# balkce/beamform

Hardware: AMD Instinct MI355X
Metric: stft_frames_per_sec (higher is better)
Workload: dtype f64; 1 GPU; das 8-mic 1024-pt (hop 512), 65536-frame batch per GPU, 1 stream(s), planar input resident in HBM; frames_per_gpu=65536, frames_fed_per_gpu=65536, mics=8, fft=1024, hop=512, streams=1, layout=planar, gather=n/a, parallelism=independent batches x1, input=uniform noise in [-0.5, 0.5), settle_launches_before_warmup=408, forward_transforms_per_frame_pair=6

## Files before the change

beamform_amd/csrc/das_f64_plan.hpp:

```cpp
#pragma once

#include <cstdlib>
#include <cstring>

#if defined(__HIPCC__)
#define BF_PLAN_HD __host__ __device__ inline
#else
#define BF_PLAN_HD inline
#endif

namespace bf {

constexpr int kChunkEnd = 0xFFFFF;
constexpr int kMaxChunkPairs = 1000;
constexpr int kSchedMaxChunks = 16384;

struct DasSchedPlan {
    int n_levels;
    int cnt[8], size[8];
    int n_chunks;
    int grid;
};

BF_PLAN_HD void das_f64_chunk(const DasSchedPlan &p, long n_frames, int n_streams, int k, int *stream, long *t0, long *n) {
    int lvl = 0, kk = k;
    long pair0 = 0;
    while (lvl < p.n_levels - 1 && kk >= p.cnt[lvl] * n_streams) {
        kk -= p.cnt[lvl] * n_streams;
        pair0 += (long)p.cnt[lvl] * p.size[lvl];
        ++lvl;
    }
    const int s = kk / p.cnt[lvl], j = kk - s * p.cnt[lvl];
    *stream = s;
    *t0 = 2 * (pair0 + (long)j * p.size[lvl]);
    long len = 2L * p.size[lvl];
    if (*t0 + len > n_frames) len = n_frames - *t0;
    *n = len;
}

inline DasSchedPlan das_f64_plan(long n_frames, int n_streams, int n_cus, const char *env) {
    DasSchedPlan p{};
    const long pairs = (n_frames + 1) / 2;
    long nb = (long)n_cus / n_streams;
    if (nb < 1) nb = 1;
    int sizes[8], n_sizes = 0;
    const long share = (pairs + nb - 1) / nb;
    if (env && strchr(env, ',')) {
        const char *c = env;
        while (*c && n_sizes < 8) {
            sizes[n_sizes++] = atoi(c);
            c = strchr(c, ',');
            if (!c) break;
            ++c;
        }
    } else if (!(env && atoi(env) == 0) && share >= 48) {
        long front = (share * 13 / 16) & ~7L;
        long rest = share - front;
        while (front > kMaxChunkPairs && n_sizes < 3) {
            sizes[n_sizes++] = kMaxChunkPairs;
            front -= kMaxChunkPairs;
        }
        if (front > kMaxChunkPairs) { rest += front - kMaxChunkPairs; front = kMaxChunkPairs; }
        sizes[n_sizes++] = (int)front;
        while (n_sizes < 6 && rest >= 24) {
            long sz = (rest / 2) & ~7L;
            if (sz > kMaxChunkPairs) sz = kMaxChunkPairs;
            sizes[n_sizes++] = (int)sz;
            rest -= sz;
        }
        if (rest >= 12) { sizes[n_sizes++] = 4; rest -= 4; }
        sizes[n_sizes++] = 2;
// ... 33 lines not shown
```

beamform_amd/csrc/das_f64_w64.hip:

```cpp
#include <hip/hip_runtime.h>

#include <type_traits>

#include "launch_trace.hpp"
#include "pipeline_kernels.hpp"
#include "switches.hpp"
#include "w64_f64_dev.hpp"

namespace bf {

namespace {

constexpr int kBlock = 512;
constexpr int kWaves = kBlock / 64;
constexpr int kHop = 512;
constexpr int kTwD = 2 * (1024 + 4 * kTw2RowW64Rot);
constexpr int oTw = 0;
constexpr int oPlane = kTwD;
constexpr int oGain = oPlane + kWaves * kPlaneD;
constexpr int oCross = oGain + 4 * 2048;
constexpr int oFlag = oCross + 512;
constexpr int kWinRow = 18;
constexpr int oWin = oFlag + 8;
constexpr int kLdsD = oWin + 64 * kWinRow;
// ... 218 lines not shown
                for (int j = 0; j < 8; ++j) atomicAdd(yo + (unsigned)(64 * j + lane), o[j]);
            }
        } else {
            const float *parea = (pw < kWaves - 1) ? reinterpret_cast<const float *>(lds + oPlane + pw * kPlaneD) : s_cross + ((it + 1) & 1) * kHop;
            while (s_ready[pw] < (int)(t - 1)) __builtin_amdgcn_s_sleep(1);
            asm volatile("" ::: "memory");
            float prev[8];
#pragma unroll
            for (int j = 0; j < 8; ++j) prev[j] = parea[64 * j + lane];
            asm volatile("" ::: "memory");
            if (lane == 0) s_cons[pw] = (int)(t - 1);
#pragma unroll
            for (int j = 0; j < 8; ++j) yo[(unsigned)(64 * j + lane)] = prev[j] + o[j];
        }
        if (t == T1 - 1) {
            if (T1 < a.n_frames) {
                float *yn = ys + T1 * kHop;
#pragma unroll
                for (int j = 0; j < 8; ++j) atomicAdd(yn + (unsigned)(64 * j + lane), o[j + 8]);
            } else {
                float *to = a.tail_out + (long)stream * kHop;
#pragma unroll
                for (int j = 0; j < 8; ++j) to[(unsigned)(64 * j + lane)] = o[j + 8];
            }
        }
    }
}


#ifdef BF_PARK_PLAIN
#define BF_PARK_LD(p) (*(const volatile float *)(p))
#else
#define BF_PARK_LD(p) __builtin_nontemporal_load(p)
#endif
constexpr int kGRow = 65;
constexpr int kGMic = 8 * kGRow;
constexpr int kSlots = 64;
constexpr int kTwP = 2 * (960 + 4 * kTw2RowW64Rot);
constexpr int pTw = 0;
constexpr int pPlane = kTwP;
constexpr int pGain = pPlane + kWaves * kPlaneD;
constexpr int pFlag = pGain + 7 * kGMic * 2;
constexpr int kRingR = 32;
constexpr int kRingSlots = kRingR + kWaves;
constexpr int pRing = pFlag + (kSlots + 4) / 2;
constexpr int pWin = pRing + kRingR / 2;
constexpr int kLdsP = pWin + 64 * kWinRow;
static_assert(kLdsP * 8 <= 160 * 1024, "LDS");
static_assert((pGain & 1) == 0 && (pWin & 1) == 0, "16-byte alignment");


typedef volatile __attribute__((address_space(3))) int *lds_int_t;
typedef volatile __attribute__((address_space(3))) unsigned long long *lds_u64_t;
__device__ __forceinline__ int lds_fetch_add(lds_int_t p, int v, int lane) {
    int old = 0;
    if (lane == 0) old = __hip_atomic_fetch_add((__attribute__((address_space(3))) int *)p, v, __ATOMIC_RELAXED, __HIP_MEMORY_SCOPE_WORKGROUP);
    return __builtin_amdgcn_readfirstlane(old);
}
__device__ __forceinline__ unsigned long long lds_fetch_add64(lds_u64_t p, int lane) {
    unsigned long long old = 0;
    if (lane == 0) old = __hip_atomic_fetch_add((__attribute__((address_space(3))) unsigned long long *)p, 1ull, __ATOMIC_RELAXED, __HIP_MEMORY_SCOPE_WORKGROUP);
    const unsigned lo = (unsigned)__builtin_amdgcn_readfirstlane((int)(unsigned)old), hi = (unsigned)__builtin_amdgcn_readfirstlane((int)(unsigned)(old >> 32));
    return ((unsigned long long)hi << 32) | lo;
}
struct DasSched {
    const int4 *chunks;
    unsigned *counter;
    int n_chunks;
};
__device__ __forceinline__ unsigned long long pack_work(unsigned vbase, int chunk, int pairs, int next) {
    return ((unsigned long long)(vbase & 0xFFFFFFu) << 40) | ((unsigned long long)(unsigned)chunk << 20) | ((unsigned long long)(unsigned)pairs << 10) | (unsigned)next;
}
struct PairWork {
    int4 d;
    int pos;
    int len;
    unsigned u;
    bool have;
};
__device__ __forceinline__ int4 load_chunk(const int4 *chunks, int k) {
    const int4 d = chunks[k];
    return int4{__builtin_amdgcn_readfirstlane(d.x), __builtin_amdgcn_readfirstlane(d.y), __builtin_amdgcn_readfirstlane(d.z), k};
}
__device__ __forceinline__ PairWork draw_pair(lds_u64_t work, const DasSched &sc, int lane, const int4 held) {
    PairWork r;
    r.have = false;
    r.d = int4{0, 0, 0, 0};
    r.pos = r.len = 0;
    r.u = 0;
    for (;;) {
        const unsigned long long old = lds_fetch_add64(work, lane);
        const int pos = (int)(old & 1023u), len = (int)((old >> 10) & 1023u), k = (int)((old >> 20) & 0xFFFFFu);
        const unsigned vb = (unsigned)(old >> 40);
        if (k == kChunkEnd) return r;
        if (pos < len) {
            if (k == held.w) r.d = held;
            else r.d = load_chunk(sc.chunks, k);
            r.pos = pos; r.len = len; r.u = vb + (unsigned)pos; r.have = true;
            return r;
        }
        if (pos == len) {
            unsigned k2 = 0;
            if (lane == 0) k2 = __hip_atomic_fetch_add(sc.counter, 1u, __ATOMIC_RELAXED, __HIP_MEMORY_SCOPE_AGENT);
            k2 = (unsigned)__builtin_amdgcn_readfirstlane((int)k2);
            if (k2 >= (unsigned)sc.n_chunks) {
                if (lane == 0) *work = pack_work(vb + (unsigned)len, kChunkEnd, 0, 0);
                return r;
            }
            r.d = load_chunk(sc.chunks, (int)k2);
            r.len = (r.d.z + 1) >> 1;
            r.pos = 0; r.u = vb + (unsigned)len; r.have = true;
            if (lane == 0) *work = pack_work(r.u, (int)k2, r.len, 1);
            return r;
        }
        while ((int)((*work >> 20) & 0xFFFFFu) == k) __builtin_amdgcn_s_sleep(2);
    }
}
__device__ __forceinline__ int claim_boundary(lds_int_t st, unsigned b, int lane) {
    const int base = 4 * (int)(b / kSlots);
    while (st[b & (kSlots - 1)] < base) __builtin_amdgcn_s_sleep(1);
    return lds_fetch_add(st + (b & (kSlots - 1)), 1, lane) - base;
}
__device__ __forceinline__ void publish_boundary(lds_int_t st, unsigned b, int lane) { (void)lds_fetch_add(st + (b & (kSlots - 1)), 2, lane); }
__device__ __forceinline__ void skip_boundary(lds_int_t st, unsigned b, int lane) {
    const int base = 4 * (int)(b / kSlots);
    while (st[b & (kSlots - 1)] < base) __builtin_amdgcn_s_sleep(1);
    (void)lds_fetch_add(st + (b & (kSlots - 1)), 4, lane);
}
__device__ __forceinline__ void await_boundary(lds_int_t st, unsigned b) {
    while (st[b & (kSlots - 1)] - 4 * (int)(b / kSlots) < 3) __builtin_amdgcn_s_sleep(1);
}

#ifdef BF_W64_STATS
__device__ unsigned long long g_stats[256 * 8 * 5];
#define BF_STATS_DECL unsigned long long st_[5] = {0, 0, 0, 0, 0}; const unsigned long long st_t0_ = __builtin_amdgcn_s_memrealtime()
#define BF_STAT(i) (++st_[i])
#define BF_STAT_WAIT_BEGIN const unsigned long long st_w0_ = __builtin_amdgcn_s_memrealtime()
#define BF_STAT_WAIT_END st_[3] += __builtin_amdgcn_s_memrealtime() - st_w0_
#define BF_STATS_FLUSH do { st_[4] = __builtin_amdgcn_s_memrealtime() - st_t0_; if (lane == 0 && blockIdx.x < 256) for (int i_ = 0; i_ < 5; ++i_) g_stats[(blockIdx.x * 8 + w) * 5 + i_] = st_[i_]; } while (0)
#else
#define BF_STATS_DECL
#define BF_STAT(i) ((void)0)
// ... 167 lines not shown
            r.h = ring_slot(jp);
        }
        __builtin_amdgcn_fence(__ATOMIC_ACQUIRE, "workgroup");
        return r;
    };
    auto release_pair = [&](const PairWork &pw, bool has_t) {
        const unsigned u2 = 2u * pw.u;
        (void)lds_fetch_add(s_ring + (u2 & (kRingR - 1)), 2, lane);
        (void)lds_fetch_add(s_ring + ((u2 + 1) & (kRingR - 1)), has_t ? 1 : 2, lane);
        if (pw.pos > 0) (void)lds_fetch_add(s_ring + ((u2 - 1) & (kRingR - 1)), 1, lane);
    };
    auto request_ring_mic = [&](const RingHops &r, int m) { request(r.h + m * kHop, r.a + m * kHop, r.b + m * kHop); };
    auto request_ring_extra = [&](bool on, const RingHops &r) {
        if (!on) {
#pragma unroll
            for (int j = 0; j < 8; ++j) e0[j] = e1[j] = e2[j] = 0.f;
            return;
        }
#pragma unroll
        for (int j = 0; j < 8; ++j) {
            e0[j] = r.h[XM * kHop + (unsigned)(64 * j + lane)];
            e1[j] = r.a[XM * kHop + (unsigned)(64 * j + lane)];
            e2[j] = r.b[XM * kHop + (unsigned)(64 * j + lane)];
        }
    };
    RingHops curR{nullptr, nullptr, nullptr};
    (void)curR;

    BF_STAMP(0);
#ifdef BF_W64_STAMPS
    if (lane == 0 && blockIdx.x < 256) g_stamps[(blockIdx.x * 8 + w) * 64 + 59] = __builtin_amdgcn_s_memtime();
#endif
    PairWork cur;
    cur.d = load_chunk(sc.chunks, (int)blockIdx.x);
    cur.len = (cur.d.z + 1) >> 1;
    const int n_static = cur.len < kWaves ? cur.len : kWaves;
    cur.pos = w;
    cur.u = (unsigned)w;
    cur.have = w < n_static;
    if (LAYOUT == 0 && cur.have) {
        request_pair_mic(cur.d.x, cur.d.y + 2L * w, a.slot_mic[0]);
        request_extra(XM >= 0, cur.d.x, cur.d.y + 2L * w);
    } else {
        request_extra(false, 0, 0);
    }
    {
        const f64x2 *tw2 = a.tw + 64;
        f64x2 *ltw = reinterpret_cast<f64x2 *>(lds + pTw), *lg = reinterpret_cast<f64x2 *>(lds + pGain);
#pragma unroll 4
        for (int i = tid; i < kTwP / 2; i += kBlock) ltw[i] = tw2[i];
        for (int k = 0; k < NT; ++k) {
            const f64x2 *g2 = a.gains_mic + a.slot_mic[k] * kGMic;
#pragma unroll 2
            for (int i = tid; i < kGMic; i += kBlock) lg[k * kGMic + i] = g2[i];
        }
#pragma unroll 2
        for (int i = tid; i < 1024; i += kBlock) lds[pWin + (i & 63) * kWinRow + (i >> 6)] = a.win[i];
        if (tid < kSlots) s_state[tid] = 0;
        if (tid < kRingR) s_ring[tid] = 0;
        if (tid == 0) *s_work = pack_work(0u, (int)blockIdx.x, cur.len, n_static);
    }
    __syncthreads();
    BF_STAMP(1);
    BF_STATS_DECL;
    int it = 0;
    if (!cur.have) {
        cur = draw_pair(s_work, sc, lane, cur.d);
// ... 184 lines not shown
        if (has_t) {
            oT = claim_boundary(s_state, u, lane);
            if (oT == 0) {
#pragma unroll
                for (int j = 0; j < 8; ++j) yn[(unsigned)(64 * j + lane)] = tl[j];
            }
        } else {
            skip_boundary(s_state, u, lane);
        }
#pragma unroll
        for (int j = 0; j < 16; ++j) {
            const float f = (float)Sr[j];
            oA[j] = (float)((double)f * wrow[j]);
        }
        if (pair) {
            float *y1 = ys + (tA + 1) * kHop;
#pragma unroll
            for (int j = 0; j < 8; ++j) {
                const float f0 = (float)Si[j];
                const float b0 = (float)((double)f0 * wrow[j]);
                y1[(unsigned)(64 * j + lane)] = oA[j + 8] + b0;
            }
        }
        if (has_h) {
            oH = claim_boundary(s_state, u - 1, lane);
            if (oH == 0) {
#pragma unroll
                for (int j = 0; j < 8; ++j) yo[(unsigned)(64 * j + lane)] = oA[j];
            }
        } else if (T0 == 0) {
            const float *ti = a.tail_in + (long)stream * kHop;
#pragma unroll
            for (int j = 0; j < 8; ++j) yo[(unsigned)(64 * j + lane)] = ti[(unsigned)(64 * j + lane)] + oA[j];
        } else {
#pragma unroll
            for (int j = 0; j < 8; ++j) atomicAdd(yo + (unsigned)(64 * j + lane), oA[j]);
        }
        if (oT == 0 || oH == 0) {
            __builtin_amdgcn_fence(__ATOMIC_RELEASE, "workgroup");
            if (oT == 0) publish_boundary(s_state, u, lane);
            if (oH == 0) publish_boundary(s_state, u - 1, lane);
        }
        if (oT > 0) {
            BF_STAT(2);
            BF_STAT_WAIT_BEGIN;
            await_boundary(s_state, u);
            BF_STAT_WAIT_END;
            __builtin_amdgcn_fence(__ATOMIC_ACQUIRE, "workgroup");
            float o[8];
#pragma unroll
            for (int j = 0; j < 8; ++j) o[j] = BF_PARK_LD(yn + (unsigned)(64 * j + lane));
#pragma unroll
            for (int j = 0; j < 8; ++j) yn[(unsigned)(64 * j + lane)] = tl[j] + o[j];
        } else {
            BF_STAT(0);
        }
        if (oH > 0) {
            BF_STAT(2);
            BF_STAT_WAIT_BEGIN;
            await_boundary(s_state, u - 1);
            BF_STAT_WAIT_END;
            __builtin_amdgcn_fence(__ATOMIC_ACQUIRE, "workgroup");
            float o[8];
#pragma unroll
            for (int j = 0; j < 8; ++j) o[j] = BF_PARK_LD(yo + (unsigned)(64 * j + lane));
#pragma unroll
            for (int j = 0; j < 8; ++j) yo[(unsigned)(64 * j + lane)] = o[j] + oA[j];
        } else {
            BF_STAT(1);
        }
        if (!has_t) {
            if (T1 < a.n_frames) {
                float *ynx = ys + T1 * kHop;
#pragma unroll
                for (int j = 0; j < 8; ++j) atomicAdd(ynx + (unsigned)(64 * j + lane), tl[j]);
            } else {
                float *to = a.tail_out + (long)stream * kHop;
#pragma unroll
                for (int j = 0; j < 8; ++j) to[(unsigned)(64 * j + lane)] = tl[j];
                if (a.hist_out != nullptr) {
                    float *ho = a.hist_out + (long)stream * M * kHop;
                    const float *xs = a.x + (long)stream * a.stream_stride_x;
                    for (int m = 0; m < M; ++m) {
                        const float *xl = xs + (long)m * a.mic_stride + tL * kHop;
#pragma unroll
                        for (int j = 0; j < 8; ++j) ho[m * kHop + 64 * j + lane] = xl[(unsigned)(64 * j + lane)];
                    }
                }
            }
        }
        if constexpr (LAYOUT == 1) {
            asm volatile("" ::: "memory");
            release_pair(cur, has_t);
        }
        cur = nxt;
        ++it;
    }
    BF_STATS_FLUSH;
#ifdef BF_W64_STAMPS
    if (lane == 0 && blockIdx.x < 256) {
        g_stamps[(blockIdx.x * 8 + w) * 64 + 63] = __builtin_amdgcn_s_memrealtime();
        g_stamps[(blockIdx.x * 8 + w) * 64 + 60] = __builtin_amdgcn_s_memtime();
        g_stamps[(blockIdx.x * 8 + w) * 64 + 62] = (unsigned long long)it;
        g_stamps[(blockIdx.x * 8 + w) * 64 + 61] = (unsigned long long)__builtin_amdgcn_s_getreg(((4 - 1) << 11) | (0 << 6) | 20);
    }
#endif
    (void)it;
}

__global__ __launch_bounds__(kBlock) void das_f64_pair_kernel(DasF64Args a, DasSched sc) { das_f64_pair_body<0>(a, sc); }
__global__ __launch_bounds__(kBlock) void das_f64_ring_kernel(DasF64Args a, DasSched sc) { das_f64_pair_body<1>(a, sc); }

constexpr int kSchedPerBlock = 8;
__global__ __launch_bounds__(32 * kSchedPerBlock) void das_f64_sched_kernel(DasSchedPlan p, int4 *chunks, unsigned *counter, float *y, long n_frames, int n_streams) {
    const int k = blockIdx.x * kSchedPerBlock + (int)(threadIdx.x >> 5), l = (int)(threadIdx.x & 31);
    if (k >= p.n_chunks) return;
    int stream;
    long t0, n;
    das_f64_chunk(p, n_frames, n_streams, k, &stream, &t0, &n);
    if (l == 0) {
        chunks[k] = int4{stream, (int)t0, (int)n, 0};
        if (k == 0) *counter = (unsigned)p.grid;
    }
    if (t0 > 0) {
        float4 *h = reinterpret_cast<float4 *>(y + ((long)stream * n_frames + t0) * kHop);
        for (int i = l; i < kHop / 4; i += 32) h[i] = float4{0.f, 0.f, 0.f, 0.f};
    }
}

__global__ __launch_bounds__(256) void interleaved_to_planar_kernel(const float *x, float *out, long tiles_per_stream, int M, long in_stream_stride,
                                                                    long out_mic_stride, long out_stream_stride) {
    __shared__ float s_t[256 * 9];
    const int tid = threadIdx.x;
    const long s = blockIdx.x / tiles_per_stream, tile = blockIdx.x - s * tiles_per_stream;
    const float4 *src = reinterpret_cast<const float4 *>(x + s * in_stream_stride + tile * 256 * M);
    const int R = M + 1;
    for (int i = tid; i < 64 * M; i += 256) {
        const float4 v = src[i];
        const int e = 4 * i;
        s_t[(e / M) * R + e % M] = v.x;
        s_t[((e + 1) / M) * R + (e + 1) % M] = v.y;
        s_t[((e + 2) / M) * R + (e + 2) % M] = v.z;
        s_t[((e + 3) / M) * R + (e + 3) % M] = v.w;
    }
    __syncthreads();
    float *dst = out + s * out_stream_stride + tile * 256;
    for (int j = tid; j < 64 * M; j += 256) {
        const int m = j >> 6, q = j & 63;
        const float4 v{s_t[(4 * q) * R + m], s_t[(4 * q + 1) * R + m], s_t[(4 * q + 2) * R + m], s_t[(4 * q + 3) * R + m]};
        reinterpret_cast<float4 *>(dst + (long)m * out_mic_stride)[q] = v;
    }
}

}

constexpr size_t kSchedCounterBytes = 256;
size_t das_f64_sched_ws_bytes() { return kSchedCounterBytes + (size_t)kSchedMaxChunks * sizeof(int4); }

DasF64Launch das_f64_decide(int layout, int n_mics, int n_streams, long n_frames, int n_cus, bool mic0_unit, int n_tr, bool tables) {
    DasF64Launch d{};
    if (n_mics > 8) return d;
    const bool ring = switches().das_il_ring != 0 && (n_mics == 2 || n_mics == 4 || n_mics == 8);
    bool frame_pair = tables && mic0_unit && n_mics >= 2 && n_tr >= 1;
    if (layout != BF_PLANAR && !ring && ((n_frames * kHop) & 255) != 0) frame_pair = false;
    if (!frame_pair) {
        if (layout == BF_PLANAR) return d;
        const long runs = n_cus > n_streams ? n_cus / n_streams : 1;
        d.path = DasF64Path::kMicPair;
        d.run_frames = ((n_frames + runs - 1) / runs + kWaves - 1) / kWaves * kWaves;
        d.runs_per_stream = (n_frames + d.run_frames - 1) / d.run_frames;
        return d;
    }
    if ((long)n_streams * ((n_frames + 1) / 2) >= (1L << 31)) return d;
    d.plan = das_f64_plan(n_frames, n_streams, n_cus, switches().das_f64_sched);
    if (d.plan.n_chunks < 1 || d.plan.n_chunks > kSchedMaxChunks) return d;
    d.path = layout == BF_PLANAR ? DasF64Path::kFramePair : ring ? DasF64Path::kRing : DasF64Path::kTranspose;
    d.writes_hist = layout == BF_PLANAR;
    const size_t hop_elems = (size_t)n_mics * kHop;
    d.scratch_bytes = sizeof(float) * (layout == BF_PLANAR ? 0 : ring ? n_cus * kRingSlots * hop_elems : n_streams * hop_elems * (n_frames + 1));
    return d;
}

static hipError_t launch_interleaved_to_planar(const float *x, float *out, long n, int n_mics, int n_streams, hipStream_t s) {
    const long tiles = n / 256;
    BF_LAUNCH(interleaved_to_planar_kernel, dim3((unsigned)(tiles * n_streams)), dim3(256), 0, s, x, out, tiles, n_mics, (long)n_mics * n, n, (long)n_mics * n);
    return hipGetLastError();
}

hipError_t enqueue_das_f64(DasF64Args a, const DasF64Launch &d, float *scratch, hipStream_t s, hipEvent_t kev0, hipEvent_t kev1, bool *kev_recorded) {
    hipError_t e = hipSuccess;
    int4 *const chunks = reinterpret_cast<int4 *>(reinterpret_cast<char *>(a.sched_ws) + kSchedCounterBytes);
    const DasSched sc{chunks, reinterpret_cast<unsigned *>(a.sched_ws), d.plan.n_chunks};
    if (d.path == DasF64Path::kMicPair) {
        for (int st = 0; st < a.n_streams && d.runs_per_stream > 1; ++st) {
            e = hipMemset2DAsync(a.y + ((long)st * a.n_frames + d.run_frames) * kHop, (size_t)d.run_frames * kHop * sizeof(float), 0, kHop * sizeof(float), (size_t)d.runs_per_stream - 1, s);
            if (e != hipSuccess) return e;
        }
    } else {
        if (d.path == DasF64Path::kRing) {
            a.ring = scratch; a.ring_bytes = d.scratch_bytes; a.hist_out = nullptr;
        } else if (d.path == DasF64Path::kTranspose) {
            const long n = a.n_frames * kHop;
            float *const hist = scratch + (size_t)a.n_streams * a.n_mics * n;
            if ((e = launch_interleaved_to_planar(a.x, scratch, n, a.n_mics, a.n_streams, s)) != hipSuccess) return e;
            if ((e = launch_interleaved_to_planar(a.hist, hist, kHop, a.n_mics, a.n_streams, s)) != hipSuccess) return e;
            a.x = scratch; a.hist = hist; a.hist_out = nullptr; a.mic_stride = n; a.layout = BF_PLANAR;
        }
        BF_LAUNCH(das_f64_sched_kernel, dim3((unsigned)((sc.n_chunks + kSchedPerBlock - 1) / kSchedPerBlock)), dim3(32 * kSchedPerBlock), 0, s, d.plan, chunks, sc.counter, a.y, a.n_frames, a.n_streams);
        if ((e = hipGetLastError()) != hipSuccess) return e;
    }
    if (kev0 && (e = hipEventRecord(kev0, s)) != hipSuccess) return e;
    if (d.path == DasF64Path::kMicPair)
        BF_LAUNCH(das_f64_w64_kernel<1>, dim3((unsigned)(d.runs_per_stream * a.n_streams)), dim3(kBlock), 0, s, a, (int)d.run_frames, (int)d.runs_per_stream);
    else if (d.path == DasF64Path::kRing)
        BF_LAUNCH(das_f64_ring_kernel, dim3((unsigned)d.plan.grid), dim3(kBlock), 0, s, a, sc);
    else
        BF_LAUNCH(das_f64_pair_kernel, dim3((unsigned)d.plan.grid), dim3(kBlock), 0, s, a, sc);
    if ((e = hipGetLastError()) != hipSuccess) return e;
    if (kev1 && (e = hipEventRecord(kev1, s)) == hipSuccess) *kev_recorded = true;
    return e;
}

}

#ifdef BF_W64_STATS
extern "C" int bf_dbg_stats(unsigned long long *host) {
    return (int)hipMemcpyFromSymbol(host, HIP_SYMBOL(bf::g_stats), sizeof(unsigned long long) * 256 * 8 * 5);
}
#endif
#ifdef BF_W64_STAMPS
extern "C" int bf_dbg_stamps(unsigned long long *host) {
    return (int)hipMemcpyFromSymbol(host, HIP_SYMBOL(bf::g_stamps), sizeof(unsigned long long) * 256 * 8 * 64);
}
#endif
```

beamform_amd/csrc/pipeline.hip:

```cpp
#include "pipeline.hpp"

#include <hip/hip_runtime.h>

#include <cmath>
#include <vector>

#include "device_mem.hpp"
#include "fft1024.hpp"
#include "pipeline_kernels.hpp"
#include "switches.hpp"

namespace bf {

namespace {

class BinPipelineImpl : public Engine {
    static constexpr int kMaxCols = BF_MAX_INTERF + 1;
   public:
    BinPipelineImpl(const bf_config &c, int n_cus) : cfg_(c), n_cus_(n_cus) {
        M_ = c.n_mics;
        H_ = c.hop;
        N_ = 2 * c.hop;
        NQ_ = problems_per_frame(N_);
        YS_ = yh_stride(N_);
// ... 28 lines not shown
        if (cov_node_ && (Phist_ < 1 || Phist_ > 64)) {
            err_ = "past_windows must be in 1..64";
            return BF_EINVAL;
        }
        if (time_node_ && (M_ > 16 || cfg_.gsc_filter_size < 1 || cfg_.gsc_filter_size > 256)) {
            err_ = "gsc is built for up to 16 microphones and filter_size 1..256";
            return M_ > 16 ? BF_ENOSYS : BF_EINVAL;
        }
        if (cfg_.algo == BF_PHASEMPF && (cfg_.smooth_size < 1 || cfg_.smooth_size > 64)) {
            err_ = "smooth_size must be in 1..64";
            return BF_EINVAL;
        }
        ENGINE_HIP(d_tw_.upload(N_ == 1024 ? twiddle_table_32x32<f64x2>() : stockham_twiddles<f64x2>(N_)));
        ENGINE_HIP(d_tw32_.upload(twiddle_table_32x32<f32x2>()));
        ENGINE_HIP(d_win_.upload(sqrt_hann(N_)));
        freqs_ = frequency_vector(N_, cfg_.sample_rate);
        ENGINE_HIP(d_freq_.upload(freqs_));
        skip_lo_ = N_; band_yh_hi_ = NQ_ - 1;
        if (band_node_) {
            int klo = N_, khi = 0;
            for (int q = 1; q < NQ_; ++q) {
                const double f = std::fabs(freqs_[q]);
                if (f >= cfg_.freq_min && f <= cfg_.freq_max) { if (q < klo) klo = q; khi = q; }
            }
            if (khi < N_ / 2 - 2) { skip_lo_ = khi; skip_hi_ = N_ - khi; }
            if (cov_node_ && khi < N_ / 2 - 1 && klo <= khi) { band_yh_lo_ = klo; band_yh_hi_ = khi; }
            else if (cov_node_ && klo > khi) { band_yh_lo_ = 1; band_yh_hi_ = 0; }
        }
        for (auto &b : d_steer_) ENGINE_HIP(b.alloc(steer_elems()));
        if (das_one_launch_shape()) {
            for (auto &b : d_dasg_w64_) ENGINE_HIP(b.alloc((size_t)4 * 1024));
            for (auto &b : d_dasg_mic_) ENGINE_HIP(b.alloc((size_t)8 * kDasMicGainRows * kDasMicGainRow));
            ENGINE_HIP(d_das_sched_.alloc(das_f64_sched_ws_bytes()));
        }
        if (N_ == 1024) ENGINE_HIP(d_tw_w64_.upload(twiddle_table_w64_rot()));
        for (auto &b : d_hist2_) ENGINE_HIP(b.alloc(hist_elems()));
        for (auto &b : d_tail_) ENGINE_HIP(b.alloc(tail_elems()));
        if (Phist_ > 0) ENGINE_HIP(d_zhist_.alloc(zhist_bytes()));
        if (cfg_.algo == BF_GSS) {
            ENGINE_HIP(d_gssW_.alloc(gss_bytes() / sizeof(f64x2)));
            ENGINE_HIP(hipMemset(d_gssW_.get(), 0, gss_bytes()));
        }
        if (cfg_.algo == BF_PHASEMPF || cfg_.algo == BF_MCRA) ENGINE_HIP(d_mpf_.alloc(mpf_bytes() / sizeof(double)));
        if (cfg_.algo == BF_PHASEMPF) ENGINE_HIP(d_smooth_.alloc(smooth_bytes() / sizeof(double)));
        if (time_node_) ENGINE_HIP(d_nlms_.alloc(nlms_bytes() / sizeof(float)));
        return BF_OK;
    }

    int reset(hipStream_t st) override {
        ENGINE_HIP(hipMemsetAsync(d_hist2_[0].get(), 0, hist_elems() * sizeof(float), st));
        hist_cur_ = 0;
        for (auto &b : d_tail_) ENGINE_HIP(hipMemsetAsync(b.get(), 0, tail_elems() * sizeof(float), st));
        tail_cur_ = 0;
        if (d_zhist_.get()) ENGINE_HIP(hipMemsetAsync(d_zhist_.get(), 0, zhist_bytes(), st));
        if (d_mpf_.get()) ENGINE_HIP(hipMemsetAsync(d_mpf_.get(), 0, mpf_bytes(), st));
        if (d_smooth_.get()) ENGINE_HIP(hipMemsetAsync(d_smooth_.get(), 0, smooth_bytes(), st));
        if (d_nlms_.get()) ENGINE_HIP(hipMemsetAsync(d_nlms_.get(), 0, nlms_bytes(), st));
        gss_reset_mask_ = ~0ull;
        return BF_OK;
    }

    int upload_steering(const std::vector<SteeringSet> &dirs, hipStream_t stream) override {
        const int nc = dirs[0].n_cols, nd = (int)dirs.size();
        if ((size_t)nd * nc * M_ * N_ > steer_elems()) {
            err_ = "steering table larger than the device buffer";
            return BF_EINVAL;
// ... 117 lines not shown
    const bool yraw_target_ = cfg_.algo == BF_PHASEMPF || time_node_;
    int skip_lo_, skip_hi_ = 0;
    int band_yh_lo_ = 0, band_yh_hi_;
    bool z48_ = false;
    size_t zsz_ = sizeof(f64x2);
    int H_ = 512, N_ = 1024, NQ_ = 514, YS_ = 516;
    const KernelSet *ks_ = nullptr;
    long steer_dir_stride_ = 0;
    std::vector<double> freqs_;
    DeviceBuffer<f64x2> d_tw_;
    DeviceBuffer<f32x2> d_tw32_;
    DeviceBuffer<double> d_win_, d_freq_;
    DeviceBuffer<f64x2> d_steer_[2];
    DeviceBuffer<f64x2> d_dasg_w64_[2];
    DeviceBuffer<f64x2> d_tw_w64_;
    DeviceBuffer<char> d_das_sched_;
    DeviceBuffer<f64x2> d_dasg_mic_[2];
    bool das_mic0_unit_[2] = {false, false};
    DasSlots das_slots_[2];
    int steer_cur_ = 0;
    DeviceBuffer<float> d_hist2_[2];
    int hist_cur_ = 0;
    DeviceBuffer<float> d_tail_[2];
    int tail_cur_ = 0;
    DeviceBuffer<char> d_zhist_;
    DeviceBuffer<f64x2> d_gssW_;
    DeviceBuffer<double> d_mpf_;
    DeviceBuffer<double> d_smooth_;
    DeviceBuffer<float> d_nlms_;
    unsigned long long gss_reset_mask_ = ~0ull;
    DeviceBuffer<char> d_Z_;
    DeviceBuffer<char> d_Yh_;
    DeviceBuffer<float> d_yraw_;
    DeviceBuffer<float> d_planar_;
    DeviceBuffer<float> d_frames_;
};

int BinPipelineImpl::run_das_one_launch(const float *x, long F, float *y, hipStream_t stream, int layout, long mic_stride, const RunSnapshot &snap) {
    if (!das_one_launch_shape() || switches().fused_bins != 1 || snap.das_gains_w64 == nullptr) return kDeclined;
    const DasF64Launch d = das_f64_decide(layout, M_, S_, F, n_cus_, snap.das_mic0_unit, snap.das_slots.n_tr,
                                          snap.das_gains_mic != nullptr && d_das_sched_.get() != nullptr);
    if (d.path == DasF64Path::kChain) return kDeclined;
    ENGINE_HIP(d_planar_.reserve((d.scratch_bytes + sizeof(float) - 1) / sizeof(float)));
    float *const hist = d_hist2_[hist_cur_].get();
    DasF64Args da;
    da.x = x; da.hist = hist; da.hist_out = d_hist2_[hist_cur_ ^ 1].get(); da.y = y;
    da.tail_in = d_tail_[tail_cur_].get(); da.tail_out = d_tail_[tail_cur_ ^ 1].get();
    da.win = d_win_.get(); da.n_frames = F; da.mic_stride = mic_stride;
    da.stream_stride_x = (long)M_ * F * H_; da.n_streams = S_; da.n_mics = M_; da.run_len = 1;
    da.layout = layout;
    da.gains = snap.das_gains_w64; da.gains_mic = snap.das_gains_mic; da.tw = d_tw_w64_.get();
    da.mic0_unit = snap.das_mic0_unit ? 1 : 0;
    da.n_tr = snap.das_slots.n_tr; da.extra_mic = snap.das_slots.extra_mic;
    for (int k = 0; k < 8; ++k) da.slot_mic[k] = snap.das_slots.slot_mic[k];
    da.sched_ws = d_das_sched_.get(); da.sched_ws_bytes = d_das_sched_.get() ? das_f64_sched_ws_bytes() : 0;
    ENGINE_HIP(enqueue_das_f64(da, d, d_planar_.get(), stream, kev0, kev1, &kev_recorded));
    if (d.writes_hist)
        hist_cur_ ^= 1;
    else
        ENGINE_HIP(carry_last_hop(hist, x, F, H_, M_, S_, layout, mic_stride, (long)F * H_ * M_, stream));
    tail_cur_ ^= 1;
    return BF_OK;
}

int BinPipelineImpl::run(const float *x, long F, float *y, f64x2 *spectrum, hipStream_t stream, int layout, long mic_stride,
                         const RunSnapshot &snap) {
    const int rc = spectrum ? kDeclined : run_das_one_launch(x, F, y, stream, layout, mic_stride, snap);
    return rc == kDeclined ? run_chain(x, F, y, spectrum, stream, layout, mic_stride, snap) : rc;
}

int BinPipelineImpl::run_chain(const float *x, long F, float *y, f64x2 *spectrum, hipStream_t stream, int layout, long mic_stride,
                               const RunSnapshot &snap) {
    const Switches &sw = switches();
    const ChainPlan p = chain_decide(ChainShape{cfg_.algo, N_, layout, M_, S_, cfg_.n_dirs > 1 ? cfg_.n_dirs : 1, snap.kp1, cfg_.past_windows,
                                                cfg_.precision, spectrum != nullptr, F, n_cus_, cfg_.gsc_filter_size, cfg_.smooth_size,
                                                band_yh_lo_, band_yh_hi_, (reinterpret_cast<size_t>(y) & 15) == 0, sw.fused_bins,
                                                sw.stft_small, sw.stft_split, sw.mvdr_group, sw.gss_group, sw.gsc_serial, R_});
    float *const hist = d_hist2_[hist_cur_].get();
    const long FT = Phist_ + F;
    ENGINE_HIP(d_Z_.reserve(p.z_bytes));
    ENGINE_HIP(d_Yh_.reserve(p.yh_bytes));
    ENGINE_HIP(d_yraw_.reserve(p.yraw_elems));
    ENGINE_HIP(d_frames_.reserve(p.frames_elems));
    f64x2 *const Z = (f64x2 *)d_Z_.get();
    f64x2 *const Yh = (f64x2 *)d_Yh_.get();
    const size_t frame_elems = (size_t)NP_ * N_;

    if (Phist_ > 0)
// ... 70 lines not shown
```

beamform_amd/csrc/pipeline_kernels.hpp:

```cpp
#pragma once

#include <hip/hip_runtime.h>

#include "../../include/bfcore.h"
#include "chain_plan.hpp"
#include "das_f64_plan.hpp"
#include "geometry.hpp"

namespace bf {

#ifdef BF_NFFT
#define BF_CAT2_(a, b) a##b
#define BF_CAT2(a, b) BF_CAT2_(a, b)
#define BF_NTAG BF_CAT2(n, BF_NFFT)
#endif

constexpr int problems_per_frame(int nfft) { return nfft / 2 + 2; }
constexpr int yh_stride(int nfft) { return nfft / 2 + 4; }
constexpr int kMpfVecs = 7;
#ifdef BF_NFFT
namespace BF_NTAG {
constexpr int kN = BF_NFFT;
constexpr int kHop = kN / 2;
constexpr int kNQ = problems_per_frame(kN);
// ... 54 lines not shown
    int yh_lo, yh_hi;
    float *y;
    const float *tail_in;
    float *tail_out;
    const f64x2 *tw;
    const f32x2 *tw32;
    const f64x2 *tw_w64 = nullptr;
    float *frames;
    const double *win;
    long n_frames;
    int n_streams;
    double post_amp;
    int use_post_amp;
};
struct DasF64Args {
    const float *x;
    const float *hist;
    float *y;
    const float *tail_in;
    float *tail_out;
    const f64x2 *gains;
    const f64x2 *tw;
    const double *win;
    long n_frames, mic_stride, stream_stride_x;
    int n_streams, n_mics, run_len;
    int layout = 0;
    float *hist_out = nullptr;
    const f64x2 *gains_mic = nullptr;
    int n_tr = 0, extra_mic = -1;
    int slot_mic[8] = {1, 2, 3, 4, 5, 6, 7, 0};
    int mic0_unit = 0;
    void *sched_ws = nullptr;
    size_t sched_ws_bytes = 0;
    float *ring = nullptr;
    size_t ring_bytes = 0;
};

enum class DasF64Path {
    kChain,
    kFramePair,
    kRing,
    kTranspose,
    kMicPair,
};
struct DasF64Launch {
    DasF64Path path;
    DasSchedPlan plan;
    long run_frames, runs_per_stream;
    size_t scratch_bytes;
    bool writes_hist;
};
DasF64Launch das_f64_decide(int layout, int n_mics, int n_streams, long n_frames, int n_cus, bool mic0_unit, int n_tr, bool tables);
hipError_t enqueue_das_f64(DasF64Args a, const DasF64Launch &d, float *scratch, hipStream_t s, hipEvent_t kev0, hipEvent_t kev1, bool *kev_recorded);
size_t das_f64_sched_ws_bytes();

#ifdef BF_NFFT
namespace BF_NTAG {
hipError_t launch_stft(const ChainPlan &p, const StftArgs &a, int n_cus, hipStream_t s);
hipError_t launch_bins(const ChainPlan &p, const BinsArgs &a, int n_cus, hipStream_t s);
hipError_t launch_stft_bins_fused(const ChainPlan &p, const StftArgs &a, const BinsArgs &b, int n_cus, hipStream_t s);
hipError_t launch_pointwise(const ChainPlan &p, const BinsArgs &a, hipStream_t s);
hipError_t launch_mpf_mask(const ChainPlan &p, const BinsArgs &a, hipStream_t s);
hipError_t launch_mcra_node(const BinsArgs &a, hipStream_t s);
hipError_t launch_mvdr_lcmv(const ChainPlan &p, const BinsArgs &a, int n_cus, hipStream_t s);
hipError_t launch_gss(const ChainPlan &p, const BinsArgs &a, hipStream_t s);
hipError_t launch_gsc_align(const BinsArgs &a, hipStream_t s);
// ... 40 lines not shown
```

Measured before the change: 135.6 million frames/s.

## Replace scheduler prep kernel and atomic overlap-add with edge tickets

Removes the separate scheduling kernel, which precomputed the chunk table and zeroed the chunk-head output rows. Chunk descriptors are now computed on the fly from the plan, and the work counter resets itself when the last block exits. Boundary overlap-add between chunks no longer uses float atomicAdd into zeroed output. Each side writes its half into an edge buffer and takes a per-chunk ticket, and the second arriver sums both halves and stores the result. This drops one kernel launch and the zeroing traffic, but adds fences, ticket atomics and an extra edge buffer.

Result: slower. 80.42 million frames/s (-40.7%).

```diff
diff --git a/beamform_amd/csrc/das_f64_plan.hpp b/beamform_amd/csrc/das_f64_plan.hpp
--- a/beamform_amd/csrc/das_f64_plan.hpp
+++ b/beamform_amd/csrc/das_f64_plan.hpp
@@ -1,5 +1,6 @@
 #pragma once
 
+#include <cstddef>
 #include <cstdlib>
 #include <cstring>
 
@@ -37,6 +38,25 @@
     if (*t0 + len > n_frames) len = n_frames - *t0;
     *n = len;
 }
+
+BF_PLAN_HD int das_f64_chunk_after(const DasSchedPlan &p, int n_streams, int k) {
+    int lvl = 0, kk = k, row0 = 0;
+    while (lvl < p.n_levels - 1 && kk >= p.cnt[lvl] * n_streams) {
+        kk -= p.cnt[lvl] * n_streams;
+        row0 += p.cnt[lvl] * n_streams;
+        ++lvl;
+    }
+    const int s = kk / p.cnt[lvl], j = kk - s * p.cnt[lvl];
+    if (j + 1 < p.cnt[lvl]) return k + 1;
+    if (lvl + 1 >= p.n_levels) return -1;
+    return row0 + p.cnt[lvl] * n_streams + s * p.cnt[lvl + 1];
+}
+
+constexpr size_t kSchedStateBytes = 256 + sizeof(int) * (size_t)kSchedMaxChunks;
+constexpr int kEdgeHop = 512;
+BF_PLAN_HD bool das_f64_edge_second(int old_ticket) { return (old_ticket & 1) != 0; }
+BF_PLAN_HD bool das_f64_last_block_out(unsigned old_done, int grid) { return old_done == (unsigned)(grid - 1); }
+inline size_t das_f64_edge_elems(int n_chunks) { return (size_t)n_chunks * 2 * kEdgeHop; }
 
 inline DasSchedPlan das_f64_plan(long n_frames, int n_streams, int n_cus, const char *env) {
     DasSchedPlan p{};
diff --git a/beamform_amd/csrc/das_f64_w64.hip b/beamform_amd/csrc/das_f64_w64.hip
--- a/beamform_amd/csrc/das_f64_w64.hip
+++ b/beamform_amd/csrc/das_f64_w64.hip
@@ -274,6 +274,17 @@
 #define BF_PARK_LD(p) (*(const volatile float *)(p))
 #else
 #define BF_PARK_LD(p) __builtin_nontemporal_load(p)
+#endif
+#ifdef BF_EDGE_SC1
+#define BF_EDGE_ST(p, v) __hip_atomic_store(p, v, __ATOMIC_RELAXED, __HIP_MEMORY_SCOPE_AGENT)
+#define BF_EDGE_RELEASE() ((void)0)
+#define BF_EDGE_TICKET_ORDER __ATOMIC_RELAXED
+#define BF_EDGE_ACQUIRE() __builtin_amdgcn_fence(__ATOMIC_ACQUIRE, "agent")
+#else
+#define BF_EDGE_ST(p, v) (*(p) = (v))
+#define BF_EDGE_RELEASE() __threadfence()
+#define BF_EDGE_TICKET_ORDER __ATOMIC_ACQ_REL
+#define BF_EDGE_ACQUIRE() ((void)0)
 #endif
 constexpr int kGRow = 65;
 constexpr int kGMic = 8 * kGRow;
@@ -306,9 +317,12 @@
     return ((unsigned long long)hi << 32) | lo;
 }
 struct DasSched {
-    const int4 *chunks;
+    DasSchedPlan plan;
+    long n_frames;
+    int n_streams;
     unsigned *counter;
-    int n_chunks;
+    int *ticket;
+    float *edge;
 };
 __device__ __forceinline__ unsigned long long pack_work(unsigned vbase, int chunk, int pairs, int next) {
     return ((unsigned long long)(vbase & 0xFFFFFFu) << 40) | ((unsigned long long)(unsigned)chunk << 20) | ((unsigned long long)(unsigned)pairs << 10) | (unsigned)next;
@@ -320,9 +334,11 @@
     unsigned u;
     bool have;
 };
-__device__ __forceinline__ int4 load_chunk(const int4 *chunks, int k) {
-    const int4 d = chunks[k];
-    return int4{__builtin_amdgcn_readfirstlane(d.x), __builtin_amdgcn_readfirstlane(d.y), __builtin_amdgcn_readfirstlane(d.z), k};
+__device__ __forceinline__ int4 load_chunk(const DasSched &sc, int k) {
+    int stream;
+    long t0, n;
+    das_f64_chunk(sc.plan, sc.n_frames, sc.n_streams, k, &stream, &t0, &n);
+    return int4{stream, (int)t0, (int)n, k};
 }
 __device__ __forceinline__ PairWork draw_pair(lds_u64_t work, const DasSched &sc, int lane, const int4 held) {
     PairWork r;
@@ -337,19 +353,26 @@
         if (k == kChunkEnd) return r;
         if (pos < len) {
             if (k == held.w) r.d = held;
-            else r.d = load_chunk(sc.chunks, k);
+            else r.d = load_chunk(sc, k);
             r.pos = pos; r.len = len; r.u = vb + (unsigned)pos; r.have = true;
             return r;
         }
         if (pos == len) {
             unsigned k2 = 0;
             if (lane == 0) k2 = __hip_atomic_fetch_add(sc.counter, 1u, __ATOMIC_RELAXED, __HIP_MEMORY_SCOPE_AGENT);
-            k2 = (unsigned)__builtin_amdgcn_readfirstlane((int)k2);
-            if (k2 >= (unsigned)sc.n_chunks) {
+            k2 = (unsigned)sc.plan.grid + (unsigned)__builtin_amdgcn_readfirstlane((int)k2);
+            if (k2 >= (unsigned)sc.plan.n_chunks) {
                 if (lane == 0) *work = pack_work(vb + (unsigned)len, kChunkEnd, 0, 0);
+                if (lane == 0) {
+                    const unsigned gone = __hip_atomic_fetch_add(sc.counter + 32, 1u, __ATOMIC_ACQ_REL, __HIP_MEMORY_SCOPE_AGENT);
+                    if (das_f64_last_block_out(gone, sc.plan.grid)) {
+                        __hip_atomic_store(sc.counter, 0u, __ATOMIC_RELAXED, __HIP_MEMORY_SCOPE_AGENT);
+                        __hip_atomic_store(sc.counter + 32, 0u, __ATOMIC_RELAXED, __HIP_MEMORY_SCOPE_AGENT);
+                    }
+                }
                 return r;
             }
-            r.d = load_chunk(sc.chunks, (int)k2);
+            r.d = load_chunk(sc, (int)k2);
             r.len = (r.d.z + 1) >> 1;
             r.pos = 0; r.u = vb + (unsigned)len; r.have = true;
             if (lane == 0) *work = pack_work(r.u, (int)k2, r.len, 1);
@@ -583,7 +606,7 @@
     if (lane == 0 && blockIdx.x < 256) g_stamps[(blockIdx.x * 8 + w) * 64 + 59] = __builtin_amdgcn_s_memtime();
 #endif
     PairWork cur;
-    cur.d = load_chunk(sc.chunks, (int)blockIdx.x);
+    cur.d = load_chunk(sc, (int)blockIdx.x);
     cur.len = (cur.d.z + 1) >> 1;
     const int n_static = cur.len < kWaves ? cur.len : kWaves;
     cur.pos = w;
@@ -834,9 +857,6 @@
             const float *ti = a.tail_in + (long)stream * kHop;
 #pragma unroll
             for (int j = 0; j < 8; ++j) yo[(unsigned)(64 * j + lane)] = ti[(unsigned)(64 * j + lane)] + oA[j];
-        } else {
-#pragma unroll
-            for (int j = 0; j < 8; ++j) atomicAdd(yo + (unsigned)(64 * j + lane), oA[j]);
         }
         if (oT == 0 || oH == 0) {
             __builtin_amdgcn_fence(__ATOMIC_RELEASE, "workgroup");
@@ -871,12 +891,47 @@
         } else {
             BF_STAT(1);
         }
+        const bool edge_h = !has_h && T0 > 0, edge_t = !has_t && T1 < a.n_frames;
+        if (edge_h || edge_t) {
+            const int kh = cur.d.w, kt = edge_t ? das_f64_chunk_after(sc.plan, sc.n_streams, cur.d.w) : -1;
+            const bool ok_t = edge_t && (unsigned)kt < (unsigned)sc.plan.n_chunks;
+            float *eh = sc.edge + (size_t)kh * (2 * kHop), *et = sc.edge + (size_t)(ok_t ? kt : 0) * (2 * kHop);
+            if (edge_h) {
+#pragma unroll
+                for (int j = 0; j < 8; ++j) BF_EDGE_ST(eh + kHop + (unsigned)(64 * j + lane), oA[j]);
+            }
+            if (ok_t) {
+#pragma unroll
+                for (int j = 0; j < 8; ++j) BF_EDGE_ST(et + (unsigned)(64 * j + lane), tl[j]);
+            }
+            BF_EDGE_RELEASE();
+            asm volatile("s_waitcnt vmcnt(0)" ::: "memory");
+            int th = 0, tt = 0;
+            if (lane == 0) {
+                if (edge_h) th = __hip_atomic_fetch_add(sc.ticket + kh, 1, BF_EDGE_TICKET_ORDER, __HIP_MEMORY_SCOPE_AGENT);
+                if (ok_t) tt = __hip_atomic_fetch_add(sc.ticket + kt, 1, BF_EDGE_TICKET_ORDER, __HIP_MEMORY_SCOPE_AGENT);
+            }
+            const bool sum_h = edge_h && das_f64_edge_second(__builtin_amdgcn_readfirstlane(th));
+            const bool sum_t = ok_t && das_f64_edge_second(__builtin_amdgcn_readfirstlane(tt));
+            if (sum_h || sum_t) BF_EDGE_ACQUIRE();
+            if (sum_h) {
+                float o[8];
+#pragma unroll
+                for (int j = 0; j < 8; ++j) o[j] = BF_PARK_LD(eh + (unsigned)(64 * j + lane));
+#pragma unroll
+                for (int j = 0; j < 8; ++j) yo[(unsigned)(64 * j + lane)] = o[j] + oA[j];
+            }
+            if (sum_t) {
+                float *ynx = ys + T1 * kHop;
+                float o[8];
+#pragma unroll
+                for (int j = 0; j < 8; ++j) o[j] = BF_PARK_LD(et + kHop + (unsigned)(64 * j + lane));
+#pragma unroll
+                for (int j = 0; j < 8; ++j) ynx[(unsigned)(64 * j + lane)] = tl[j] + o[j];
+            }
+        }
         if (!has_t) {
-            if (T1 < a.n_frames) {
-                float *ynx = ys + T1 * kHop;
-#pragma unroll
-                for (int j = 0; j < 8; ++j) atomicAdd(ynx + (unsigned)(64 * j + lane), tl[j]);
-            } else {
+            if (!(T1 < a.n_frames)) {
                 float *to = a.tail_out + (long)stream * kHop;
 #pragma unroll
                 for (int j = 0; j < 8; ++j) to[(unsigned)(64 * j + lane)] = tl[j];
@@ -912,23 +967,6 @@
 
 __global__ __launch_bounds__(kBlock) void das_f64_pair_kernel(DasF64Args a, DasSched sc) { das_f64_pair_body<0>(a, sc); }
 __global__ __launch_bounds__(kBlock) void das_f64_ring_kernel(DasF64Args a, DasSched sc) { das_f64_pair_body<1>(a, sc); }
-
-constexpr int kSchedPerBlock = 8;
-__global__ __launch_bounds__(32 * kSchedPerBlock) void das_f64_sched_kernel(DasSchedPlan p, int4 *chunks, unsigned *counter, float *y, long n_frames, int n_streams) {
-    const int k = blockIdx.x * kSchedPerBlock + (int)(threadIdx.x >> 5), l = (int)(threadIdx.x & 31);
-    if (k >= p.n_chunks) return;
-    int stream;
-    long t0, n;
-    das_f64_chunk(p, n_frames, n_streams, k, &stream, &t0, &n);
-    if (l == 0) {
-        chunks[k] = int4{stream, (int)t0, (int)n, 0};
-        if (k == 0) *counter = (unsigned)p.grid;
-    }
-    if (t0 > 0) {
-        float4 *h = reinterpret_cast<float4 *>(y + ((long)stream * n_frames + t0) * kHop);
-        for (int i = l; i < kHop / 4; i += 32) h[i] = float4{0.f, 0.f, 0.f, 0.f};
-    }
-}
 
 __global__ __launch_bounds__(256) void interleaved_to_planar_kernel(const float *x, float *out, long tiles_per_stream, int M, long in_stream_stride,
                                                                     long out_mic_stride, long out_stream_stride) {
@@ -956,8 +994,7 @@
 
 }
 
-constexpr size_t kSchedCounterBytes = 256;
-size_t das_f64_sched_ws_bytes() { return kSchedCounterBytes + (size_t)kSchedMaxChunks * sizeof(int4); }
+size_t das_f64_sched_ws_bytes() { return kSchedStateBytes; }
 
 DasF64Launch das_f64_decide(int layout, int n_mics, int n_streams, long n_frames, int n_cus, bool mic0_unit, int n_tr, bool tables) {
     DasF64Launch d{};
@@ -991,8 +1028,10 @@
 
 hipError_t enqueue_das_f64(DasF64Args a, const DasF64Launch &d, float *scratch, hipStream_t s, hipEvent_t kev0, hipEvent_t kev1, bool *kev_recorded) {
     hipError_t e = hipSuccess;
-    int4 *const chunks = reinterpret_cast<int4 *>(reinterpret_cast<char *>(a.sched_ws) + kSchedCounterBytes);
-    const DasSched sc{chunks, reinterpret_cast<unsigned *>(a.sched_ws), d.plan.n_chunks};
+    char *const ws = reinterpret_cast<char *>(a.sched_ws);
+    const DasSched sc{d.plan, a.n_frames, a.n_streams, reinterpret_cast<unsigned *>(ws), reinterpret_cast<int *>(ws + 256), a.sched_edge};
+    if (d.path != DasF64Path::kMicPair && (a.sched_ws_bytes < kSchedStateBytes || a.sched_edge_bytes < das_f64_edge_elems(d.plan.n_chunks) * sizeof(float)))
+        return hipErrorInvalidValue;
     if (d.path == DasF64Path::kMicPair) {
         for (int st = 0; st < a.n_streams && d.runs_per_stream > 1; ++st) {
             e = hipMemset2DAsync(a.y + ((long)st * a.n_frames + d.run_frames) * kHop, (size_t)d.run_frames * kHop * sizeof(float), 0, kHop * sizeof(float), (size_t)d.runs_per_stream - 1, s);
@@ -1008,8 +1047,6 @@
             if ((e = launch_interleaved_to_planar(a.hist, hist, kHop, a.n_mics, a.n_streams, s)) != hipSuccess) return e;
             a.x = scratch; a.hist = hist; a.hist_out = nullptr; a.mic_stride = n; a.layout = BF_PLANAR;
         }
-        BF_LAUNCH(das_f64_sched_kernel, dim3((unsigned)((sc.n_chunks + kSchedPerBlock - 1) / kSchedPerBlock)), dim3(32 * kSchedPerBlock), 0, s, d.plan, chunks, sc.counter, a.y, a.n_frames, a.n_streams);
-        if ((e = hipGetLastError()) != hipSuccess) return e;
     }
     if (kev0 && (e = hipEventRecord(kev0, s)) != hipSuccess) return e;
     if (d.path == DasF64Path::kMicPair)
diff --git a/beamform_amd/csrc/pipeline.hip b/beamform_amd/csrc/pipeline.hip
--- a/beamform_amd/csrc/pipeline.hip
+++ b/beamform_amd/csrc/pipeline.hip
@@ -84,6 +84,7 @@
             for (auto &b : d_dasg_w64_) ENGINE_HIP(b.alloc((size_t)4 * 1024));
             for (auto &b : d_dasg_mic_) ENGINE_HIP(b.alloc((size_t)8 * kDasMicGainRows * kDasMicGainRow));
             ENGINE_HIP(d_das_sched_.alloc(das_f64_sched_ws_bytes()));
+            ENGINE_HIP(hipMemset(d_das_sched_.get(), 0, das_f64_sched_ws_bytes()));
         }
         if (N_ == 1024) ENGINE_HIP(d_tw_w64_.upload(twiddle_table_w64_rot()));
         for (auto &b : d_hist2_) ENGINE_HIP(b.alloc(hist_elems()));
@@ -267,6 +268,7 @@
     DeviceBuffer<char> d_Z_;
     DeviceBuffer<char> d_Yh_;
     DeviceBuffer<float> d_yraw_;
+    DeviceBuffer<float> d_das_edge_;
     DeviceBuffer<float> d_planar_;
     DeviceBuffer<float> d_frames_;
 };
@@ -277,6 +279,7 @@
                                           snap.das_gains_mic != nullptr && d_das_sched_.get() != nullptr);
     if (d.path == DasF64Path::kChain) return kDeclined;
     ENGINE_HIP(d_planar_.reserve((d.scratch_bytes + sizeof(float) - 1) / sizeof(float)));
+    if (d.path != DasF64Path::kMicPair) ENGINE_HIP(d_das_edge_.reserve(das_f64_edge_elems(d.plan.n_chunks)));
     float *const hist = d_hist2_[hist_cur_].get();
     DasF64Args da;
     da.x = x; da.hist = hist; da.hist_out = d_hist2_[hist_cur_ ^ 1].get(); da.y = y;
@@ -289,6 +292,7 @@
     da.n_tr = snap.das_slots.n_tr; da.extra_mic = snap.das_slots.extra_mic;
     for (int k = 0; k < 8; ++k) da.slot_mic[k] = snap.das_slots.slot_mic[k];
     da.sched_ws = d_das_sched_.get(); da.sched_ws_bytes = d_das_sched_.get() ? das_f64_sched_ws_bytes() : 0;
+    da.sched_edge = d_das_edge_.get(); da.sched_edge_bytes = d_das_edge_.size() * sizeof(float);
     ENGINE_HIP(enqueue_das_f64(da, d, d_planar_.get(), stream, kev0, kev1, &kev_recorded));
     if (d.writes_hist)
         hist_cur_ ^= 1;
diff --git a/beamform_amd/csrc/pipeline_kernels.hpp b/beamform_amd/csrc/pipeline_kernels.hpp
--- a/beamform_amd/csrc/pipeline_kernels.hpp
+++ b/beamform_amd/csrc/pipeline_kernels.hpp
@@ -110,6 +110,8 @@
     int mic0_unit = 0;
     void *sched_ws = nullptr;
     size_t sched_ws_bytes = 0;
+    float *sched_edge = nullptr;
+    size_t sched_edge_bytes = 0;
     float *ring = nullptr;
     size_t ring_bytes = 0;
 };
```
